# zssjh/stereo-semantic-vo

Measured on AMD Instinct MI355X. Metric: stereo frames/sec on KITTI 00 (full Tracking::Track chain), higher is better.
Workload: dtype u8; 1 GPU; BASELINE configs[2]: synth-kitti00 sequence of 4541 distinct 1241x376 stereo pairs, full Tracking::Track loop per frame (ORB on L and R, sparse stereo, matching passes 1+2, PnP-RANSAC, pose-only LM, map-point lifecycle); ONE sequence per GPU in strict frame order (replicas across GPUs); parallelism=one GPU, resident_pairs_per_gpu=4541, resident_input_bytes_per_gpu=4370984960, frames_tracked=4541, tracker_capacity_flag=0, pnp_samples_through_sequential_fallback=0

## Files before the change

stereo-semantic-vo_amd/csrc/svo_epnp_ord_dev.h:

```cpp
#pragma once
#ifndef HIP_INCLUDE_HIP_HIP_RUNTIME_H
#include <hip/hip_runtime.h>
#endif
#include <stdint.h>

#include "svo_epnp_exact_dev.h"

namespace epnp_ord {

#define EO_FN __device__ __forceinline__
typedef double d2 __attribute__((ext_vector_type(2)));

#include "svo_epnp_ord_tab.h"
#include "svo_epnp_ord_asm.h"

#define EO_SYNC()                                         \
  do {                                                    \
    __builtin_amdgcn_fence(__ATOMIC_ACQ_REL, "wavefront"); \
    __builtin_amdgcn_wave_barrier();                      \
  } while (0)

struct Lds {
  alignas(16) double jr[16 * 16];
  alignas(16) double xch[16][4][4];
  unsigned tab[EO_TAB_TOTAL];
  double pws[16], us[10], alphas[20], cws[12], ccinv[9];
  double M[120];
  double ut4[4][12];
  double L[60], rho[6];
  double sw[3][6];
  double bx[3][6];
  double ccs[3][12], pcs[3][16], abt[3][9], Rc[3][9], rep[3][8];
  alignas(16) double gn[3][6][6];
  double out[3][16];
  int srow[3][6];
  int urow[4];
  double xw[16];
  int flag;
  int sweeps;
  int why;
  long long stamp[8];
#ifdef EO_PROFILE
  long long prof[8];
#endif
};

EO_FN double xdiv(double a, double b) { return a / b; }
EO_FN double xsqrt(double x) { return sqrt(x); }

EO_FN double ndiv(double a, double b) {
  double r = __builtin_amdgcn_rcp(b);
  double e = __builtin_fma(-b, r, 1.0);
  r = __builtin_fma(r, e, r);
  e = __builtin_fma(-b, r, 1.0);
  r = __builtin_fma(r, e, r);
  const double q = a * r;
  const double rem = __builtin_fma(-b, q, a);
  return __builtin_fma(rem, r, q);
}
EO_FN double nsqrt(double x) {
  const double y = __builtin_amdgcn_rsq(x);
  double g = x * y, h = 0.5 * y;
  const double r = __builtin_fma(-h, g, 0.5);
  g = __builtin_fma(g, r, g);
  h = __builtin_fma(h, r, h);
  double d = __builtin_fma(-g, g, x);
  g = __builtin_fma(d, h, g);
  d = __builtin_fma(-g, g, x);
  g = __builtin_fma(d, h, g);
  return g;
}
EO_FN bool w_in_range(double w) { return w >= 7.888609052210118e-31 && w <= 1.2676506002282294e30; }

EO_FN double gsum(double term, double acc) { return __builtin_amdgcn_mfma_f64_4x4x4f64(1.0, term, acc, 0, 0, 0); }
template <int M>
EO_FN double colsum(double t0, double t1, double t2, int g) {
  double acc = gsum(M >= 4 || g < M ? t0 : 0.0, 0.0);
  if (M > 4) acc = gsum(M >= 8 || 4 + g < M ? t1 : 0.0, acc);
  if (M > 8) acc = gsum(M >= 12 || 8 + g < M ? t2 : 0.0, acc);
  return acc;
}

#define EO_TAB3_OFF 0
#define EO_TAB4_OFF (EO_TAB3_OFF + EO_TAB3_STEPS * 3)
#define EO_TAB5_OFF (EO_TAB4_OFF + EO_TAB4_STEPS * 4)
#define EO_TAB12_OFF (EO_TAB5_OFF + EO_TAB5_STEPS * 5)
EO_FN unsigned tab_entry(unsigned e) { return (e & ~16u) | ((e & 16u) << 27); }
EO_FN void load_tables(Lds& S, int lane) {
  for (int e = lane; e < EO_TAB3_STEPS * 3; e += 64) S.tab[EO_TAB3_OFF + e] = tab_entry(c_tab3[0][e]);
  for (int e = lane; e < EO_TAB4_STEPS * 4; e += 64) S.tab[EO_TAB4_OFF + e] = tab_entry(c_tab4[0][e]);
  for (int e = lane; e < EO_TAB5_STEPS * 5; e += 64) S.tab[EO_TAB5_OFF + e] = tab_entry(c_tab5[0][e]);
  for (int e = lane; e < EO_TAB12_STEPS * 12; e += 64) S.tab[EO_TAB12_OFF + e] = tab_entry(c_tab12[0][e]);
}

template <int M>
EO_FN void pair_test(double x0, double x1, double x2, double q0, double q1, double q2, double W, double wP, double mk,
                     double& p, double& thr) {
  const double one = 1.0, eps = 2.220446049250313e-16 * 10;
  double t0, t1, t2, ab, y, g, h, r, d;
  if (M == 12) {
    asm volatile(
        "v_mul_f64 %[t0], %[x0], %[q0]\n\t"
        "v_mul_f64 %[ab], %[W], %[wP]\n\t"
        "v_mul_f64 %[t1], %[x1], %[q1]\n\t"
        "v_mul_f64 %[t2], %[x2], %[q2]\n\t"
        "v_rsq_f64 %[y], %[ab]\n\t"
        "v_mfma_f64_4x4x4_4b_f64 %[p], %[one], %[t0], 0\n\t"
        "v_mul_f64 %[g], %[ab], %[y]\n\t"
        "v_mul_f64 %[h], %[y], 0.5\n\t"
        "v_fma_f64 %[r], -%[h], %[g], 0.5\n\t"
        "v_fma_f64 %[g], %[g], %[r], %[g]\n\t"
        "v_mfma_f64_4x4x4_4b_f64 %[p], %[one], %[t1], %[p]\n\t"
        "v_fma_f64 %[h], %[h], %[r], %[h]\n\t"
        "v_fma_f64 %[d], -%[g], %[g], %[ab]\n\t"
        "v_fma_f64 %[g], %[d], %[h], %[g]\n\t"
        "v_fma_f64 %[d], -%[g], %[g], %[ab]\n\t"
        "v_mfma_f64_4x4x4_4b_f64 %[p], %[one], %[t2], %[p]\n\t"
        "v_fma_f64 %[g], %[d], %[h], %[g]\n\t"
        "v_mul_f64 %[thr], %[g], %[eps]\n\t"
        "s_nop 4"
        : [p] "=&v"(p), [thr] "=&v"(thr), [t0] "=&v"(t0), [t1] "=&v"(t1), [t2] "=&v"(t2), [ab] "=&v"(ab), [y] "=&v"(y),
          [g] "=&v"(g), [h] "=&v"(h), [r] "=&v"(r), [d] "=&v"(d)
        : [x0] "v"(x0), [x1] "v"(x1), [x2] "v"(x2), [q0] "v"(q0), [q1] "v"(q1), [q2] "v"(q2), [W] "v"(W), [wP] "v"(wP),
          [one] "v"(one), [eps] "v"(eps));
  } else if (M == 6) {
    asm volatile(
        "v_mul_f64 %[t0], %[x0], %[q0]\n\t"
        "v_mul_f64 %[t1], %[x1], %[q1]\n\t"
        "v_mul_f64 %[ab], %[W], %[wP]\n\t"
        "v_mul_f64 %[t1], %[t1], %[mk]\n\t"
        "v_rsq_f64 %[y], %[ab]\n\t"
        "v_mfma_f64_4x4x4_4b_f64 %[p], %[one], %[t0], 0\n\t"
        "v_mul_f64 %[g], %[ab], %[y]\n\t"
        "v_mul_f64 %[h], %[y], 0.5\n\t"
        "v_fma_f64 %[r], -%[h], %[g], 0.5\n\t"
        "v_fma_f64 %[g], %[g], %[r], %[g]\n\t"
        "v_mfma_f64_4x4x4_4b_f64 %[p], %[one], %[t1], %[p]\n\t"
        "v_fma_f64 %[h], %[h], %[r], %[h]\n\t"
        "v_fma_f64 %[d], -%[g], %[g], %[ab]\n\t"
        "v_fma_f64 %[g], %[d], %[h], %[g]\n\t"
        "v_fma_f64 %[d], -%[g], %[g], %[ab]\n\t"
        "v_fma_f64 %[g], %[d], %[h], %[g]\n\t"
        "v_mul_f64 %[thr], %[g], %[eps]\n\t"
        "s_nop 0"
        : [p] "=&v"(p), [thr] "=&v"(thr), [t0] "=&v"(t0), [t1] "=&v"(t1), [ab] "=&v"(ab), [y] "=&v"(y), [g] "=&v"(g),
          [h] "=&v"(h), [r] "=&v"(r), [d] "=&v"(d)
        : [x0] "v"(x0), [x1] "v"(x1), [q0] "v"(q0), [q1] "v"(q1), [W] "v"(W), [wP] "v"(wP), [mk] "v"(mk), [one] "v"(one),
          [eps] "v"(eps));
  } else {
    asm volatile(
        "v_mul_f64 %[t0], %[x0], %[q0]\n\t"
        "v_mul_f64 %[ab], %[W], %[wP]\n\t"
        "v_mul_f64 %[t0], %[t0], %[mk]\n\t"
        "v_rsq_f64 %[y], %[ab]\n\t"
        "s_nop 0\n\t"
        "v_mfma_f64_4x4x4_4b_f64 %[p], %[one], %[t0], 0\n\t"
        "v_mul_f64 %[g], %[ab], %[y]\n\t"
        "v_mul_f64 %[h], %[y], 0.5\n\t"
        "v_fma_f64 %[r], -%[h], %[g], 0.5\n\t"
        "v_fma_f64 %[g], %[g], %[r], %[g]\n\t"
        "v_fma_f64 %[h], %[h], %[r], %[h]\n\t"
        "v_fma_f64 %[d], -%[g], %[g], %[ab]\n\t"
        "v_fma_f64 %[g], %[d], %[h], %[g]\n\t"
        "v_fma_f64 %[d], -%[g], %[g], %[ab]\n\t"
        "v_fma_f64 %[g], %[d], %[h], %[g]\n\t"
        "v_mul_f64 %[thr], %[g], %[eps]"
        : [p] "=&v"(p), [thr] "=&v"(thr), [t0] "=&v"(t0), [ab] "=&v"(ab), [y] "=&v"(y), [g] "=&v"(g), [h] "=&v"(h), [r] "=&v"(r),
          [d] "=&v"(d)
        : [x0] "v"(x0), [q0] "v"(q0), [W] "v"(W), [wP] "v"(wP), [mk] "v"(mk), [one] "v"(one), [eps] "v"(eps));
  }
}

template <int M>
EO_FN double row_norm2(double n0, double n1, double n2, double mk) {
  const double one = 1.0;
  double s0, s1, s2, a;
  if (M == 12) {
    asm volatile(
        "v_mul_f64 %[s0], %[n0], %[n0]\n\t"
        "v_mul_f64 %[s1], %[n1], %[n1]\n\t"
        "v_mul_f64 %[s2], %[n2], %[n2]\n\t"
        "v_mfma_f64_4x4x4_4b_f64 %[a], %[one], %[s0], 0\n\t"
        "s_nop 3\n\t"
        "v_mfma_f64_4x4x4_4b_f64 %[a], %[one], %[s1], %[a]\n\t"
        "s_nop 3\n\t"
        "v_mfma_f64_4x4x4_4b_f64 %[a], %[one], %[s2], %[a]\n\t"
        "s_nop 5"
        : [a] "=&v"(a), [s0] "=&v"(s0), [s1] "=&v"(s1), [s2] "=&v"(s2)
        : [n0] "v"(n0), [n1] "v"(n1), [n2] "v"(n2), [one] "v"(one));
  } else if (M == 6) {
    asm volatile(
        "v_mul_f64 %[s0], %[n0], %[n0]\n\t"
        "v_mul_f64 %[s1], %[n1], %[n1]\n\t"
        "v_mul_f64 %[s1], %[s1], %[mk]\n\t"
        "v_mfma_f64_4x4x4_4b_f64 %[a], %[one], %[s0], 0\n\t"
        "s_nop 3\n\t"
        "v_mfma_f64_4x4x4_4b_f64 %[a], %[one], %[s1], %[a]\n\t"
        "s_nop 5"
        : [a] "=&v"(a), [s0] "=&v"(s0), [s1] "=&v"(s1)
        : [n0] "v"(n0), [n1] "v"(n1), [mk] "v"(mk), [one] "v"(one));
  } else {
    asm volatile(
        "v_mul_f64 %[s0], %[n0], %[n0]\n\t"
        "v_mul_f64 %[s0], %[s0], %[mk]\n\t"
        "s_nop 1\n\t"
        "v_mfma_f64_4x4x4_4b_f64 %[a], %[one], %[s0], 0\n\t"
        "s_nop 5"
        : [a] "=&v"(a), [s0] "=&v"(s0)
        : [n0] "v"(n0), [mk] "v"(mk), [one] "v"(one));
  }
  return a;
}

template <int M>
EO_FN unsigned long long jacobi_rows(Lds& S, int n, int base, int lane) {
  const int r = lane & 15, g = lane >> 4, q = r - base;
  const double mk = M == 6 ? (g < 2 ? 1.0 : 0.0) : (M == 3 ? (g < 3 ? 1.0 : 0.0) : 1.0);
  const double eps = 2.220446049250313e-16 * 10;
  double x0 = S.jr[r * 16 + g], x1 = S.jr[r * 16 + 4 + g], x2 = S.jr[r * 16 + 8 + g];
  double* const mine = S.xch[r][g];
  { d2 lo; lo.x = x0; lo.y = x1; *reinterpret_cast<d2*>(mine) = lo; mine[2] = x2; }
  const int tb = n == 12 ? EO_TAB12_OFF : (n == 5 ? EO_TAB5_OFF : (n == 4 ? EO_TAB4_OFF : EO_TAB3_OFF));
  const int steps = n == 12 ? EO_TAB12_STEPS : (n == 5 ? EO_TAB5_STEPS : (n == 4 ? EO_TAB4_STEPS : EO_TAB3_STEPS));
  const int pro = n == 12 ? EO_TAB12_PROLOGUE : (n == 5 ? EO_TAB5_PROLOGUE : (n == 4 ? EO_TAB4_PROLOGUE : EO_TAB3_PROLOGUE));
  static_assert(EO_TAB3_SWEEPS == 1 && EO_TAB4_SWEEPS == 1 && EO_TAB5_SWEEPS == 1 && EO_TAB12_SWEEPS == 1, "one sweep per period");
  auto lds = [](const void* p) { return (unsigned)(unsigned long long)p; };
  const unsigned a_tab = lds(&S.tab[0]);
  const unsigned twrap = a_tab + 4u * (unsigned)(n > 0 ? tb + pro * n + q : 0);
  const unsigned cfg = (unsigned)steps | (unsigned)pro << 8 | (unsigned)(4 * n) << 16;
  const unsigned pm = n > 0 ? ((1u << n) - 1u) << base : 0u;
  EO_SYNC();
  const double eps2 = eps * eps;
  const double eps2hi = eps2 * (1.0 + 9.094947017729282e-13), eps2lo = eps2 * (1.0 - 9.094947017729282e-13);
  unsigned chg = 0, nst = 0, flag = 0;
  int tt = 0, tp = n > 0 ? tb + q : 0, sb = 0;
  const unsigned e0 = S.tab[tp];
  ++tt; tp += n;
  if (tt == steps) { tt = pro; tp = n > 0 ? tb + pro * n + q : 0; ++sb; }
  const unsigned e1 = S.tab[tp];
  const unsigned tpa = a_tab + 4u * (unsigned)tp;
  const unsigned act = n >= 2 ? 1u : 0u;
  const unsigned amine = lds(mine), axch = lds(&S.xch[0][g][0]);
#define EO_JACOBI_OPERANDS                                                                                                       \
  : [x0] "+v"(x0), [x1] "+v"(x1), [x2] "+v"(x2), [chg] "+v"(chg), [nst] "+v"(nst), [flag] "+v"(flag)                              \
  : [e0] "v"(e0), [e1] "v"(e1), [tt] "v"(tt), [tp] "v"(tpa), [sb] "v"(sb), [cfg] "v"(cfg), [twrap] "v"(twrap), [lane] "v"(lane), \
    [base] "v"(base), [act] "v"(act), [pm] "v"(pm), [mk] "v"(mk), [eps] "v"(eps), [eps2hi] "v"(eps2hi), [eps2lo] "v"(eps2lo),   \
    [amine] "v"(amine), [axch] "v"(axch)                                                                                          \
  : EO_JACOBI_ASM_CLOBBERS
  if (M == 12) asm volatile(EO_JACOBI_ASM_12 EO_JACOBI_OPERANDS);
  else if (M == 6) asm volatile(EO_JACOBI_ASM_6 EO_JACOBI_OPERANDS);
  else asm volatile(EO_JACOBI_ASM_3 EO_JACOBI_OPERANDS);
#undef EO_JACOBI_OPERANDS
  const unsigned long long exhausted = __ballot(flag != 0 && n > 0);
  if (M == 12 && flag) S.why |= 1;
  if (M == 12 && lane == 0) S.sweeps = (int)nst;
  const double w = xsqrt(row_norm2<M>(x0, x1, x2, mk));
  const double sc1 = 1 / w;
  if (n > 0) {
    S.jr[r * 16 + g] = M >= 4 || g < M ? x0 * sc1 : x0;
    S.jr[r * 16 + 4 + g] = M >= 8 || 4 + g < M ? x1 * sc1 : x1;
    S.jr[r * 16 + 8 + g] = M >= 12 || 8 + g < M ? x2 * sc1 : x2;
    if (g == 0) S.jr[r * 16 + 15] = w;
  }
  EO_SYNC();
  return exhausted;
}

EO_FN unsigned long long svd_rank(Lds& S, int n, int base, int p, int lane) {
  const int col = lane & 15;
  bool bad = false;
  if (col < n) {
    const double my = S.jr[(base + col) * 16 + 15];
    int rank = 0;
    bad = !w_in_range(my);
    for (int q = 0; q < 5; ++q)
      if (q < n && q != col) {
        const double o = S.jr[(base + q) * 16 + 15];
        rank += o > my ? 1 : 0;
        bad = bad || o == my;
      }
    S.sw[p][rank] = my;
    S.srow[p][rank] = base + col;
  }
  EO_SYNC();
  return __ballot(bad);
}
EO_FN unsigned need_seq(unsigned long long ex, unsigned long long bad) {
  unsigned m = 0;
  for (int p = 0; p < 3; ++p) {
    const unsigned long long rows = 0x001F001F001F001FULL << (5 * p);
    if ((ex & rows) || (bad & (0xFFFFULL << (16 * p)))) m |= 1u << p;
  }
  return m;
}

EO_FN int svd12_smallest(Lds& S, int lane) {
  bool local = false, full = false;
  if (lane < 12) {
    const double my = S.jr[lane * 16 + 15];
    int rank = 0;
    local = my == 0.0;
    full = !w_in_range(my);
    for (int q = 0; q < 12; ++q)
      if (q != lane) {
        const double o = S.jr[q * 16 + 15];
        rank += o > my ? 1 : 0;
        local = local || o == my;
      }
    if (full) S.why |= 2;
    if (rank >= 8) S.urow[11 - rank] = lane;
  }
  const bool any_local = __ballot(local) != 0, any_full = __ballot(full) != 0;
  EO_SYNC();
  if (any_full) return 2;
  if (any_local) return 1;
  if (lane < 48) {
    const int q = lane / 12, k = lane % 12, r = S.urow[q] & 15;
    S.ut4[q][k] = S.jr[r * 16 + k];
  }
  EO_SYNC();
  return 0;
}

__device__ __attribute__((noinline)) void jacobi12_safe(Lds& S, int lane) {
  const double eps = 2.220446049250313e-16 * 10;
  const int r = lane & 15, g = lane >> 4, n = r < 12 ? 12 : 0, q = r;
  double x0 = S.jr[r * 16 + g], x1 = S.jr[r * 16 + 4 + g], x2 = S.jr[r * 16 + 8 + g];
  double W = colsum<12>(x0 * x0, x1 * x1, x2 * x2, g);
  double* const mine = S.xch[r][g];
  mine[0] = x0; mine[1] = x1; mine[2] = x2;
  S.xw[r] = W;
  const int tb = EO_TAB12_OFF, steps = EO_TAB12_STEPS, pro = EO_TAB12_PROLOGUE;
  const unsigned pm = n > 0 ? (1u << 12) - 1u : 0u;
  EO_SYNC();
  int tt = 0, tp = n > 0 ? tb + q : 0, sbase = 0;
  unsigned chg = 0;
  bool active = n >= 2;
  unsigned e = S.tab[tp];
  int nsteps = 0;
  while (__any(active)) {
    int tn = tt + 1, tpn = tp + n, sbn = sbase;
    if (tn == steps) { tn = pro; tpn = tb + pro * n + q; sbn = sbase + 1; }
    const unsigned en = S.tab[n > 0 ? tpn : 0];
    const int pq = e & 15, sw = sbase + (int)((e >> 5) & 3);
    const bool is_j = (e >> 31) != 0;
    const bool valid = active && pq != q && sw < 30;
    const int pr = valid ? pq : r;
    const double* const theirs = S.xch[pr][g];
    const double y0 = theirs[0], y1 = theirs[1], y2 = theirs[2];
    const double p0 = colsum<12>(x0 * y0, x1 * y1, x2 * y2, g);
    const double wP = S.xw[pr];
    const bool rot = valid && !(fabs(p0) <= eps * xsqrt(W * wP));
    if (__any(rot)) {
      const double p = p0 * 2;
      double beta = W - wP;
      if (is_j) beta = -beta;
      double gamma;
      {
        double a = fabs(p), b = fabs(beta);
        if (a > b) { b = xdiv(b, a); gamma = a * xsqrt(1 + b * b); }
        else if (b > 0) { a = xdiv(a, b); gamma = b * xsqrt(1 + a * a); }
        else gamma = 0;
      }
      double c, sn;
      if (beta < 0) {
        const double delta = (gamma - beta) * 0.5;
        sn = xsqrt(xdiv(delta, gamma));
        c = xdiv(p, gamma * sn * 2);
      } else {
        c = xsqrt(xdiv(gamma + beta, gamma * 2));
        sn = xdiv(p, gamma * c * 2);
      }
      const double se = is_j ? -sn : sn;
      const double n0 = c * x0 + se * y0, n1 = c * x1 + se * y1, n2 = c * x2 + se * y2;
      const double Wn = colsum<12>(n0 * n0, n1 * n1, n2 * n2, g);
      EO_SYNC();
      if (rot) {
        x0 = n0; x1 = n1; x2 = n2; W = Wn;
        chg |= 1u << sw;
        mine[0] = x0; mine[1] = x1; mine[2] = x2;
        S.xw[r] = W;
      }
    }
    EO_SYNC();
    const bool closes = active && (e & 0x80u) != 0;
    if (__any(closes)) {
      const int sc = sbase + (int)((e >> 8) & 3);
      const unsigned long long bal = __ballot(closes && ((chg >> (sc & 31)) & 1u));
      if (closes && (sc >= 29 || ((unsigned)bal & pm) == 0u)) active = false;
    }
    tt = tn; tp = tpn; sbase = sbn; e = en;
    ++nsteps;
  }
  if (lane == 0) S.sweeps = 1000000 + nsteps;
  EO_SYNC();
}

typedef __attribute__((address_space(3))) double lds_double;
__device__ __attribute__((noinline)) void svd_small_seq(Lds& S, double* jW, int M, int n, int base, int p) {
  double w[6];
  epnp_exact::jacobi_svd((lds_double*)jW, (lds_double*)&S.jr[base * 16], 16, w, (lds_double*)&S.jr[base * 16 + M], 16, M, n, n);
  for (int i = 0; i < n; ++i) {
    S.sw[p][i] = w[i];
    S.srow[p][i] = base + i;
    S.jr[(base + i) * 16 + 15] = w[i];
  }
  S.flag |= 2; S.why |= 8;
}

__device__ __attribute__((noinline)) void svd12_finish_seq(Lds& S, epnp_exact::Work& xw) {
  for (int i = 0; i < 12; ++i)
    for (int k = 0; k < 12; ++k) xw.ut[i * 12 + k] = S.xch[i][k & 3][k >> 2];
  epnp_exact::jacobi_svd_finish((lds_double*)xw.jW, (lds_double*)xw.ut, 12, xw.d, (lds_double*)nullptr, 0, 12, 12, 12);
  for (int q = 0; q < 4; ++q)
    for (int k = 0; k < 12; ++k) S.ut4[q][k] = xw.ut[(11 - q) * 12 + k];
  S.flag |= 2; S.why |= 4;
}

EO_FN void gauss_newton(Lds& S, int cand, int col, bool owner, const double* L, const double* rho, double* betas) {
  for (int it = 0; it < 5; ++it) {
    double A[6][4], b[6];
    {
      const int i = col < 6 ? col : 0;
      const double* rl = L + 10 * i;
      double* g = S.gn[cand][i];
      const double a0 = 2 * rl[0] * betas[0] + rl[1] * betas[1] + rl[3] * betas[2] + rl[6] * betas[3];
      const double a1 = rl[1] * betas[0] + 2 * rl[2] * betas[1] + rl[4] * betas[2] + rl[7] * betas[3];
      const double a2 = rl[3] * betas[0] + rl[4] * betas[1] + 2 * rl[5] * betas[2] + rl[8] * betas[3];
      const double a3 = rl[6] * betas[0] + rl[7] * betas[1] + rl[8] * betas[2] + 2 * rl[9] * betas[3];
      const double bi = rho[i] - (rl[0] * betas[0] * betas[0] + rl[1] * betas[0] * betas[1] + rl[2] * betas[1] * betas[1] +
                                  rl[3] * betas[0] * betas[2] + rl[4] * betas[1] * betas[2] + rl[5] * betas[2] * betas[2] +
                                  rl[6] * betas[0] * betas[3] + rl[7] * betas[1] * betas[3] + rl[8] * betas[2] * betas[3] +
                                  rl[9] * betas[3] * betas[3]);
      if (owner && col < 6) { g[0] = a0; g[1] = a1; g[2] = a2; g[3] = a3; g[4] = bi; }
    }
    EO_SYNC();
#pragma unroll
    for (int i = 0; i < 6; ++i) {
      const double* g = S.gn[cand][i];
      A[i][0] = g[0]; A[i][1] = g[1]; A[i][2] = g[2]; A[i][3] = g[3]; b[i] = g[4];
    }
    EO_SYNC();
    double A1[4], A2[4], x[4] = {0, 0, 0, 0};
    bool alive = true;
#pragma unroll
    for (int k = 0; k < 4; ++k) {
      double eta = fabs(A[k][k]);
#pragma unroll
      for (int i = k + 1; i < 6; ++i) {
        const double elt = fabs(A[i - 1][k]);
        if (eta < elt) eta = elt;
      }
      if (eta == 0) alive = false;
      const double inv_eta = 1. / eta;
      double sum2 = 0.0;
#pragma unroll
      for (int i = k; i < 6; ++i) {
        A[i][k] *= inv_eta;
        sum2 += A[i][k] * A[i][k];
      }
      double sigma = xsqrt(sum2);
      if (A[k][k] < 0) sigma = -sigma;
      A[k][k] += sigma;
      A1[k] = sigma * A[k][k];
      A2[k] = -eta * sigma;
#pragma unroll
      for (int j = k + 1; j < 4; ++j) {
        double sum = 0;
#pragma unroll
        for (int i = k; i < 6; ++i) sum += A[i][k] * A[i][j];
        const double tau = sum / A1[k];
#pragma unroll
        for (int i = k; i < 6; ++i) A[i][j] -= tau * A[i][k];
      }
    }
#pragma unroll
    for (int j = 0; j < 4; ++j) {
      double tau = 0;
#pragma unroll
      for (int i = j; i < 6; ++i) tau += A[i][j] * b[i];
      tau /= A1[j];
#pragma unroll
      for (int i = j; i < 6; ++i) b[i] -= tau * A[i][j];
    }
    x[3] = b[3] / A2[3];
#pragma unroll
    for (int i = 2; i >= 0; --i) {
      double sum = 0;
#pragma unroll
      for (int j = i + 1; j < 4; ++j) sum += A[i][j] * x[j];
      x[i] = (b[i] - sum) / A2[i];
    }
#pragma unroll
    for (int i = 0; i < 4; ++i) betas[i] += alive ? x[i] : 0.0;
  }
}

EO_FN double dot3(const double* a, const double* b) { return a[0] * b[0] + a[1] * b[1] + a[2] * b[2]; }

EO_FN bool solve5_wave(Lds& S, epnp_exact::Work& xw, const double* K, double* R_out, double* t_out, double* rep, bool force_seq = false) {
  const int lane = threadIdx.x & 63, slot = lane >> 4, col = lane & 15, r16 = lane & 15;
  const double fu = K[0], fv = K[1], uc = K[2], vc = K[3];
  if (lane == 0) { S.flag = force_seq ? 1 : 0; S.why = force_seq ? 16 : 0; S.stamp[0] = clock64(); }
  load_tables(S, lane);
  EO_SYNC();
  if (lane < 3) {
    double c = 0;
    for (int i = 0; i < 5; i++) c += S.pws[3 * i + lane];
    S.cws[lane] = c / 5;
  }
  EO_SYNC();
  auto load_pw0 = [&]() {
    if (lane < 9) {
      const int a = lane / 3, b = lane % 3;
      const double ca = S.cws[a], cb = S.cws[b];
      double s = 0;
      for (int i = 0; i < 5; ++i) s += (S.pws[3 * i + a] - ca) * (S.pws[3 * i + b] - cb);
      S.jr[b * 16 + a] = s;
    } else if (lane < 18) {
      const int r = (lane - 9) / 3, k = (lane - 9) % 3;
      S.jr[r * 16 + 3 + k] = r == k ? 1.0 : 0.0;
    } else if (lane < 36) {
      S.jr[((lane - 18) / 6) * 16 + 6 + (lane - 18) % 6] = 0.0;
    }
    EO_SYNC();
  };
  load_pw0();
  unsigned long long ex = jacobi_rows<3>(S, r16 < 3 ? 3 : 0, r16 < 3 ? 0 : r16, lane);
  unsigned long long bd = svd_rank(S, slot == 0 ? 3 : 0, 0, 0, lane);
  if (ex | bd) {
    load_pw0();
    if (lane == 0) svd_small_seq(S, xw.jW, 3, 3, 0, 0);
    EO_SYNC();
  }
  if (lane < 9) {
    const int i = 1 + lane / 3, j = lane % 3;
    const double k = xsqrt(S.sw[0][i - 1] / 5);
    S.cws[3 * i + j] = S.cws[j] + k * S.jr[S.srow[0][i - 1] * 16 + j];
  }
  EO_SYNC();
  auto load_cc = [&]() {
    if (lane < 9) {
      const int r = lane / 3, k = lane % 3;
      S.jr[r * 16 + k] = S.cws[3 * (r + 1) + k] - S.cws[k];
    } else if (lane < 18) {
      const int r = (lane - 9) / 3, k = (lane - 9) % 3;
      S.jr[r * 16 + 3 + k] = r == k ? 1.0 : 0.0;
    } else if (lane < 36) {
      S.jr[((lane - 18) / 6) * 16 + 6 + (lane - 18) % 6] = 0.0;
    }
    EO_SYNC();
  };
  load_cc();
  ex = jacobi_rows<3>(S, r16 < 3 ? 3 : 0, r16 < 3 ? 0 : r16, lane);
  bd = svd_rank(S, slot == 0 ? 3 : 0, 0, 0, lane);
  if (ex | bd) {
    load_cc();
    if (lane == 0) svd_small_seq(S, xw.jW, 3, 3, 0, 0);
    EO_SYNC();
  }
  if (lane < 9) {
    const int j = lane / 3, c = lane % 3;
    double threshold = 0;
    for (int i = 0; i < 3; ++i) threshold += S.sw[0][i];
    threshold *= 2.220446049250313e-16 * 2;
    double x = 0;
    for (int i = 0; i < 3; ++i) {
      double wi = S.sw[0][i];
      if (fabs(wi) <= threshold) continue;
      wi = 1 / wi;
      const int r = S.srow[0][i];
      double s = S.jr[r * 16 + c];
      s *= wi;
      x = x + s * S.jr[r * 16 + 3 + j];
    }
    S.ccinv[lane] = x;
  }
  EO_SYNC();
  if (lane < 15) {
    const int i = lane / 3, j = lane % 3;
    const double* ci = S.ccinv;
    const double* pi = S.pws + 3 * i;
    S.alphas[4 * i + 1 + j] = ci[3 * j] * (pi[0] - S.cws[0]) + ci[3 * j + 1] * (pi[1] - S.cws[1]) + ci[3 * j + 2] * (pi[2] - S.cws[2]);
  }
  EO_SYNC();
  if (lane < 5) {
    const double* a = S.alphas + 4 * lane;
    S.alphas[4 * lane] = 1.0f - a[1] - a[2] - a[3];
  }
  EO_SYNC();
  if (lane == 0) S.stamp[1] = clock64();
  for (int e = lane; e < 120; e += 64) {
    const int r = e / 12, cc = e % 12, i = r >> 1, q = cc / 3, t = cc % 3;
    const double as = S.alphas[4 * i + q], u = S.us[2 * i], v = S.us[2 * i + 1];
    double m;
    if (r & 1) m = t == 0 ? 0.0 : (t == 1 ? as * fv : as * (vc - v));
    else m = t == 0 ? as * fu : (t == 1 ? 0.0 : as * (uc - u));
    S.M[e] = m;
  }
  EO_SYNC();
  auto load_mtm = [&]() {
    for (int e = lane; e < 144; e += 64) {
      const int a = e / 12, b = e % 12;
      double s = 0;
      for (int r = 0; r < 10; ++r) s += S.M[12 * r + a] * S.M[12 * r + b];
      S.jr[b * 16 + a] = s;
    }
    EO_SYNC();
  };
  load_mtm();
  if (lane == 0) S.stamp[2] = clock64();
  const bool degenerate = (S.why & 8) != 0;
  unsigned long long ex12 = 0;
  int fin12 = 2;
  if (!degenerate) {
    ex12 = jacobi_rows<12>(S, r16 < 12 ? 12 : 0, r16 < 12 ? 0 : r16, lane);
    fin12 = svd12_smallest(S, lane);
  }
  if (ex12 || fin12) {
    if (ex12 || fin12 == 2) {
      if (!degenerate) load_mtm();
      jacobi12_safe(S, lane);
    }
    if (lane == 0) svd12_finish_seq(S, xw);
    EO_SYNC();
  }
  if (lane == 0) S.stamp[3] = clock64();
  if (lane < 60) {
    const int i = lane / 10, c = lane % 10;
    const int pa = i < 3 ? 0 : (i < 5 ? 1 : 2), pb = i < 3 ? i + 1 : (i < 5 ? i - 1 : 3);
    const int y = c >= 6 ? 3 : (c >= 3 ? 2 : (c >= 1 ? 1 : 0)), x = c - y * (y + 1) / 2;
    double dx[3], dy[3];
    for (int k = 0; k < 3; ++k) {
      dx[k] = S.ut4[x][3 * pa + k] - S.ut4[x][3 * pb + k];
      dy[k] = S.ut4[y][3 * pa + k] - S.ut4[y][3 * pb + k];
    }
    const double d = dot3(dx, dy);
    S.L[lane] = x == y ? d : 2.0f * d;
  }
  if (lane < 6) {
    const int pa = lane < 3 ? 0 : (lane < 5 ? 1 : 2), pb = lane < 3 ? lane + 1 : (lane < 5 ? lane - 1 : 3);
    const double* p1 = S.cws + 3 * pa;
    const double* p2 = S.cws + 3 * pb;
    S.rho[lane] = (p1[0] - p2[0]) * (p1[0] - p2[0]) + (p1[1] - p2[1]) * (p1[1] - p2[1]) + (p1[2] - p2[2]) * (p1[2] - p2[2]);
  }
  EO_SYNC();
  const int cand = slot < 3 ? slot : 0;
  const int nc = slot == 0 ? 4 : (slot == 1 ? 3 : (slot == 2 ? 5 : 0));
  const int base = 5 * cand;
  auto load_l = [&](int only) {
    if (slot < 3 && (only < 0 || slot == only)) {
      for (int i = 0; i < nc; ++i) {
        const int lc = slot == 0 ? (i == 2 ? 3 : (i == 3 ? 6 : i)) : i;
        double v = 0.0;
        if (col < 6) v = S.L[10 * col + lc];
        else if (col - 6 == i) v = 1.0;
        S.jr[(base + i) * 16 + col] = v;
      }
    }
    EO_SYNC();
  };
  load_l(-1);
  {
    const int pc = r16 / 5, pn = pc == 0 ? 4 : (pc == 1 ? 3 : 5);
    const bool mine = r16 < 15 && r16 % 5 < pn;
    ex = jacobi_rows<6>(S, mine ? pn : 0, mine ? 5 * pc : r16, lane);
  }
  bd = svd_rank(S, nc, base, cand, lane);
  if (ex | bd) {
    const unsigned need = need_seq(ex, bd);
    for (int pp = 0; pp < 3; ++pp)
      if (need >> pp & 1) load_l(pp);
    if (slot < 3 && col == 0 && (need >> slot & 1)) svd_small_seq(S, slot == 0 ? xw.jW : (slot == 1 ? xw.sA : xw.sUt), 6, nc, base, cand);
    EO_SYNC();
  }
  if (slot < 3 && col < nc) {
    double threshold = 0;
    for (int i = 0; i < nc; ++i) threshold += S.sw[cand][i];
    threshold *= 2.220446049250313e-16 * 2;
    double x = 0;
    for (int i = 0; i < nc; ++i) {
      double wi = S.sw[cand][i];
      if (fabs(wi) <= threshold) continue;
      wi = 1 / wi;
      const int r = S.srow[cand][i];
      double s = 0;
      for (int k = 0; k < 6; ++k) s += S.jr[r * 16 + k] * S.rho[k];
      s *= wi;
      x = x + s * S.jr[r * 16 + 6 + col];
    }
    S.bx[cand][col] = x;
  }
  EO_SYNC();
  if (lane == 0) S.stamp[4] = clock64();
  double betas[4];
  {
    const double* bx = S.bx[cand];
    const double b0 = bx[0], b1 = bx[1], b2 = bx[2], b3 = bx[3];
    if (slot == 0) {
      if (b0 < 0) { betas[0] = xsqrt(-b0); betas[1] = -b1 / betas[0]; betas[2] = -b2 / betas[0]; betas[3] = -b3 / betas[0]; }
      else { betas[0] = xsqrt(b0); betas[1] = b1 / betas[0]; betas[2] = b2 / betas[0]; betas[3] = b3 / betas[0]; }
    } else {
      if (b0 < 0) { betas[0] = xsqrt(-b0); betas[1] = (b2 < 0) ? xsqrt(-b2) : 0.0; }
      else { betas[0] = xsqrt(b0); betas[1] = (b2 > 0) ? xsqrt(b2) : 0.0; }
      if (b1 < 0) betas[0] = -betas[0];
      betas[2] = slot == 2 ? b3 / betas[0] : 0.0;
      betas[3] = 0.0;
    }
  }
  {
    double rho[6];
    for (int k = 0; k < 6; ++k) rho[k] = S.rho[k];
    gauss_newton(S, cand, col, slot < 3, S.L, rho, betas);
  }
  if (lane == 0) S.stamp[5] = clock64();
  if (slot < 3 && col < 12) {
    double c = 0.0;
    for (int i = 0; i < 4; ++i) c += betas[i] * S.ut4[i][col];
    S.ccs[cand][col] = c;
  }
  EO_SYNC();
  if (slot < 3 && col < 15) {
    const int i = col / 3, j = col % 3;
    const double* a = S.alphas + 4 * i;
    const double* cc = S.ccs[cand];
    S.pcs[cand][col] = a[0] * cc[j] + a[1] * cc[3 + j] + a[2] * cc[6 + j] + a[3] * cc[9 + j];
  }
  EO_SYNC();
  double pc0[3], pw0[3];
  bool flip;
  {
    const double* pc = S.pcs[cand];
    flip = pc[2] < 0.0;
    for (int j = 0; j < 3; ++j) { pc0[j] = 0; pw0[j] = 0; }
    for (int i = 0; i < 5; ++i)
      for (int j = 0; j < 3; ++j) { pc0[j] += flip ? -pc[3 * i + j] : pc[3 * i + j]; pw0[j] += S.pws[3 * i + j]; }
    for (int j = 0; j < 3; ++j) { pc0[j] /= 5; pw0[j] /= 5; }
  }
  auto load_abt = [&](int only) {
    const double* pc = S.pcs[cand];
    if (slot < 3 && (only < 0 || slot == only) && col < 9) {
      const int j = col / 3, k = col % 3;
      double s = 0;
      for (int i = 0; i < 5; ++i) s += ((flip ? -pc[3 * i + j] : pc[3 * i + j]) - pc0[j]) * (S.pws[3 * i + k] - pw0[k]);
      S.jr[(base + k) * 16 + j] = s;
    } else if (slot < 3 && (only < 0 || slot == only) && col < 12) {
      const int r = col - 9;
      for (int k = 0; k < 3; ++k) S.jr[(base + r) * 16 + 3 + k] = r == k ? 1.0 : 0.0;
      for (int k = 6; k < 12; ++k) S.jr[(base + r) * 16 + k] = 0.0;
    }
    EO_SYNC();
  };
  load_abt(-1);
  {
    const bool mine = r16 < 15 && r16 % 5 < 3;
    ex = jacobi_rows<3>(S, mine ? 3 : 0, mine ? 5 * (r16 / 5) : r16, lane);
  }
  bd = svd_rank(S, slot < 3 ? 3 : 0, base, cand, lane);
  if (ex | bd) {
    const unsigned need = need_seq(ex, bd);
    for (int pp = 0; pp < 3; ++pp)
      if (need >> pp & 1) load_abt(pp);
    if (slot < 3 && col == 0 && (need >> slot & 1)) svd_small_seq(S, slot == 0 ? xw.jW : (slot == 1 ? xw.sA : xw.sUt), 3, 3, base, cand);
    EO_SYNC();
  }
  if (slot < 3 && col < 9) {
    const int i = col / 3, j = col % 3;
    const int r0 = S.srow[cand][0], r1 = S.srow[cand][1], r2 = S.srow[cand][2];
    S.Rc[cand][col] = S.jr[r0 * 16 + i] * S.jr[r0 * 16 + 3 + j] + S.jr[r1 * 16 + i] * S.jr[r1 * 16 + 3 + j] + S.jr[r2 * 16 + i] * S.jr[r2 * 16 + 3 + j];
  }
  EO_SYNC();
  double R[9], t[3];
  for (int k = 0; k < 9; ++k) R[k] = S.Rc[cand][k];
  {
    const double det = R[0] * R[4] * R[8] + R[1] * R[5] * R[6] + R[2] * R[3] * R[7] - R[2] * R[4] * R[6] - R[1] * R[3] * R[8] - R[0] * R[5] * R[7];
    if (det < 0) { R[6] = -R[6]; R[7] = -R[7]; R[8] = -R[8]; }
  }
  t[0] = pc0[0] - dot3(R, pw0); t[1] = pc0[1] - dot3(R + 3, pw0); t[2] = pc0[2] - dot3(R + 6, pw0);
  if (slot < 3 && col < 5) {
    const double* pw = S.pws + 3 * col;
    const double Xc = dot3(R, pw) + t[0], Yc = dot3(R + 3, pw) + t[1], inv_Zc = 1.0 / (dot3(R + 6, pw) + t[2]);
    const double ue = uc + fu * Xc * inv_Zc, ve = vc + fv * Yc * inv_Zc;
    const double u = S.us[2 * col], v = S.us[2 * col + 1];
    S.rep[cand][col] = xsqrt((u - ue) * (u - ue) + (v - ve) * (v - ve));
  }
  EO_SYNC();
  if (slot < 3 && col == 0) {
    double sum2 = 0.0;
    for (int i = 0; i < 5; ++i) sum2 += S.rep[cand][i];
    double* o = S.out[cand];
    for (int k = 0; k < 9; ++k) o[k] = R[k];
    o[9] = t[0]; o[10] = t[1]; o[11] = t[2];
    o[12] = sum2 / 5;
  }
  EO_SYNC();
  if (lane == 0) S.stamp[6] = clock64();
  bool fin = true;
  if (S.flag & 1) {
    if (lane == 0) {
      double* x5 = xw.PW0;
      double* u5 = xw.gA;
      for (int i = 0; i < 15; ++i) x5[i] = S.pws[i];
      for (int i = 0; i < 10; ++i) u5[i] = S.us[i];
      double Rx[9], tx[3], rx[3];
      const bool ok = epnp_exact::solve5(xw, x5, u5, K, Rx, tx, rx);
      for (int k = 0; k < 9; ++k) S.out[0][k] = Rx[k];
      for (int k = 0; k < 3; ++k) S.out[0][9 + k] = tx[k];
      S.out[0][12] = rx[0]; S.out[1][12] = rx[1]; S.out[2][12] = rx[2];
      S.out[0][13] = ok ? 1.0 : 0.0;
    }
    EO_SYNC();
    for (int k = 0; k < 9; ++k) R_out[k] = S.out[0][k];
    for (int k = 0; k < 3; ++k) t_out[k] = S.out[0][9 + k];
    fin = S.out[0][13] != 0.0;
  } else {
    int N = 0;
    if (S.out[1][12] < S.out[0][12]) N = 1;
    if (S.out[2][12] < S.out[N][12]) N = 2;
    for (int k = 0; k < 9; ++k) { R_out[k] = S.out[N][k]; fin = fin && isfinite(S.out[N][k]); }
    for (int k = 0; k < 3; ++k) { t_out[k] = S.out[N][9 + k]; fin = fin && isfinite(S.out[N][9 + k]); }
  }
  if (rep) { rep[0] = S.out[0][12]; rep[1] = S.out[1][12]; rep[2] = S.out[2][12]; }
  if (lane == 0) S.stamp[7] = clock64();
  EO_SYNC();
  return fin;
}

}
```

Measured before the change: 9537 stereo frames/s.

## Distribute Gauss-Newton QR across row lanes with DPP broadcasts instead of LDS

Replaces the per-lane redundant Gauss-Newton 6x4 QR solve, which exchanged its rows through LDS with wave barriers each iteration, with a lane-distributed formulation. Each of the first lanes in a 16-lane row owns one column of A (or b), and pivot data is broadcast with DPP row_newbcast. This removes the LDS scratch array and the two syncs per iteration and spreads the QR arithmetic across lanes. It adds a host-side bitwise checker so the lane version can be compared against a reference. The risk is precision or ordering differences from the original serial code, plus extra broadcast instructions.

```diff
diff --git a/stereo-semantic-vo_amd/csrc/svo_epnp_ord_dev.h b/stereo-semantic-vo_amd/csrc/svo_epnp_ord_dev.h
--- a/stereo-semantic-vo_amd/csrc/svo_epnp_ord_dev.h
+++ b/stereo-semantic-vo_amd/csrc/svo_epnp_ord_dev.h
@@ -5,6 +5,7 @@
 #include <stdint.h>
 
 #include "svo_epnp_exact_dev.h"
+#include "svo_lanes.h"
 
 namespace epnp_ord {
 
@@ -31,7 +32,6 @@
   double sw[3][6];
   double bx[3][6];
   double ccs[3][12], pcs[3][16], abt[3][9], Rc[3][9], rep[3][8];
-  alignas(16) double gn[3][6][6];
   double out[3][16];
   int srow[3][6];
   int urow[4];
@@ -417,83 +417,28 @@
   S.flag |= 2; S.why |= 4;
 }
 
-EO_FN void gauss_newton(Lds& S, int cand, int col, bool owner, const double* L, const double* rho, double* betas) {
-  for (int it = 0; it < 5; ++it) {
-    double A[6][4], b[6];
-    {
-      const int i = col < 6 ? col : 0;
-      const double* rl = L + 10 * i;
-      double* g = S.gn[cand][i];
-      const double a0 = 2 * rl[0] * betas[0] + rl[1] * betas[1] + rl[3] * betas[2] + rl[6] * betas[3];
-      const double a1 = rl[1] * betas[0] + 2 * rl[2] * betas[1] + rl[4] * betas[2] + rl[7] * betas[3];
-      const double a2 = rl[3] * betas[0] + rl[4] * betas[1] + 2 * rl[5] * betas[2] + rl[8] * betas[3];
-      const double a3 = rl[6] * betas[0] + rl[7] * betas[1] + rl[8] * betas[2] + 2 * rl[9] * betas[3];
-      const double bi = rho[i] - (rl[0] * betas[0] * betas[0] + rl[1] * betas[0] * betas[1] + rl[2] * betas[1] * betas[1] +
-                                  rl[3] * betas[0] * betas[2] + rl[4] * betas[1] * betas[2] + rl[5] * betas[2] * betas[2] +
-                                  rl[6] * betas[0] * betas[3] + rl[7] * betas[1] * betas[3] + rl[8] * betas[2] * betas[3] +
-                                  rl[9] * betas[3] * betas[3]);
-      if (owner && col < 6) { g[0] = a0; g[1] = a1; g[2] = a2; g[3] = a3; g[4] = bi; }
-    }
-    EO_SYNC();
+struct RowDpp {
+  typedef double real;
+  typedef bool mask;
+  int col;
+  EO_FN double c(double d) const { return d; }
+  EO_FN double abs(double a) const { return fabs(a); }
+  EO_FN double sqrt(double a) const { return xsqrt(a); }
+  EO_FN bool lt(double a, double b) const { return a < b; }
+  EO_FN bool eq(double a, double b) const { return a == b; }
+  EO_FN double sel(bool m, double a, double b) const { return m ? a : b; }
+  EO_FN bool land(bool a, bool b) const { return a && b; }
+  EO_FN bool lnot(bool a) const { return !a; }
+  EO_FN bool lane_is(int l) const { return col == l; }
+  template <int K>
+  EO_FN double bcast(double v) const { return __builtin_amdgcn_update_dpp(v, v, 0x150 + K, 0xf, 0xf, false); }
+};
+EO_FN void gauss_newton(const Lds& S, int col, double* betas) {
+  const RowDpp x{col};
+  double coef[svo_lanes::GN_NCOEF];
 #pragma unroll
-    for (int i = 0; i < 6; ++i) {
-      const double* g = S.gn[cand][i];
-      A[i][0] = g[0]; A[i][1] = g[1]; A[i][2] = g[2]; A[i][3] = g[3]; b[i] = g[4];
-    }
-    EO_SYNC();
-    double A1[4], A2[4], x[4] = {0, 0, 0, 0};
-    bool alive = true;
-#pragma unroll
-    for (int k = 0; k < 4; ++k) {
-      double eta = fabs(A[k][k]);
-#pragma unroll
-      for (int i = k + 1; i < 6; ++i) {
-        const double elt = fabs(A[i - 1][k]);
-        if (eta < elt) eta = elt;
-      }
-      if (eta == 0) alive = false;
-      const double inv_eta = 1. / eta;
-      double sum2 = 0.0;
-#pragma unroll
-      for (int i = k; i < 6; ++i) {
-        A[i][k] *= inv_eta;
-        sum2 += A[i][k] * A[i][k];
-      }
-      double sigma = xsqrt(sum2);
-      if (A[k][k] < 0) sigma = -sigma;
-      A[k][k] += sigma;
-      A1[k] = sigma * A[k][k];
-      A2[k] = -eta * sigma;
-#pragma unroll
-      for (int j = k + 1; j < 4; ++j) {
-        double sum = 0;
-#pragma unroll
-        for (int i = k; i < 6; ++i) sum += A[i][k] * A[i][j];
-        const double tau = sum / A1[k];
-#pragma unroll
-        for (int i = k; i < 6; ++i) A[i][j] -= tau * A[i][k];
-      }
-    }
-#pragma unroll
-    for (int j = 0; j < 4; ++j) {
-      double tau = 0;
-#pragma unroll
-      for (int i = j; i < 6; ++i) tau += A[i][j] * b[i];
-      tau /= A1[j];
-#pragma unroll
-      for (int i = j; i < 6; ++i) b[i] -= tau * A[i][j];
-    }
-    x[3] = b[3] / A2[3];
-#pragma unroll
-    for (int i = 2; i >= 0; --i) {
-      double sum = 0;
-#pragma unroll
-      for (int j = i + 1; j < 4; ++j) sum += A[i][j] * x[j];
-      x[i] = (b[i] - sum) / A2[i];
-    }
-#pragma unroll
-    for (int i = 0; i < 4; ++i) betas[i] += alive ? x[i] : 0.0;
-  }
+  for (int e = 0; e < svo_lanes::GN_NCOEF; ++e) coef[e] = svo_lanes::gn_lane_coef(S.L, S.rho, col, e);
+  svo_lanes::gauss_newton_lanes(x, coef, betas);
 }
 
 EO_FN double dot3(const double* a, const double* b) { return a[0] * b[0] + a[1] * b[1] + a[2] * b[2]; }
@@ -708,11 +653,7 @@
       betas[3] = 0.0;
     }
   }
-  {
-    double rho[6];
-    for (int k = 0; k < 6; ++k) rho[k] = S.rho[k];
-    gauss_newton(S, cand, col, slot < 3, S.L, rho, betas);
-  }
+  gauss_newton(S, col, betas);
   if (lane == 0) S.stamp[5] = clock64();
   if (slot < 3 && col < 12) {
     double c = 0.0;
diff --git a/stereo-semantic-vo_amd/csrc/svo_lanes.h b/stereo-semantic-vo_amd/csrc/svo_lanes.h
--- /dev/null
+++ b/stereo-semantic-vo_amd/csrc/svo_lanes.h
@@ -0,0 +1,127 @@
+#pragma once
+
+#if defined(__HIPCC__)
+#define SVO_LANES_FN __device__ __forceinline__
+#define SVO_LANES_UNROLL _Pragma("unroll")
+#else
+#define SVO_LANES_FN inline __attribute__((always_inline))
+#define SVO_LANES_UNROLL
+#endif
+
+namespace svo_lanes {
+
+constexpr int GN_NCOEF = 24;
+SVO_LANES_FN int gn_lane_coef_index(int col, int e) {
+  const int i = e >> 2, j = e & 3, a = col < j ? col : j, b = col < j ? j : col;
+  const int in_a = 10 * i + b * (b + 1) / 2 + a;
+  const int row = col - 4;
+  const int in_b = e < 10 ? 10 * row + e : (e == 10 ? 60 + row : -1);
+  return col < 4 ? in_a : (col < 10 ? in_b : -1);
+}
+SVO_LANES_FN bool gn_lane_coef_doubled(int col, int e) { return col < 4 && (e & 3) == col; }
+SVO_LANES_FN double gn_lane_coef(const double* L, const double* rho, int col, int e) {
+  const int idx = gn_lane_coef_index(col, e);
+  const double* src = idx >= 60 ? rho + (idx - 60) : L + (idx < 0 ? 0 : idx);
+  double v = *src;
+  if (idx < 0) v = 0.0;
+  return gn_lane_coef_doubled(col, e) ? 2 * v : v;
+}
+
+template <class X>
+SVO_LANES_FN void gn_build_lanes(const X& x, const typename X::real* coef, const typename X::real* betas, typename X::real* v) {
+  typedef typename X::real R;
+  const R b0 = betas[0], b1 = betas[1], b2 = betas[2], b3 = betas[3];
+  R acol[6];
+SVO_LANES_UNROLL
+  for (int i = 0; i < 6; ++i) acol[i] = coef[4 * i] * b0 + coef[4 * i + 1] * b1 + coef[4 * i + 2] * b2 + coef[4 * i + 3] * b3;
+  const R bi = coef[10] - (coef[0] * b0 * b0 + coef[1] * b0 * b1 + coef[2] * b1 * b1 + coef[3] * b0 * b2 + coef[4] * b1 * b2 +
+                           coef[5] * b2 * b2 + coef[6] * b0 * b3 + coef[7] * b1 * b3 + coef[8] * b2 * b3 + coef[9] * b3 * b3);
+  const typename X::mask is_b = x.lane_is(4);
+  v[0] = x.sel(is_b, x.template bcast<4>(bi), acol[0]);
+  v[1] = x.sel(is_b, x.template bcast<5>(bi), acol[1]);
+  v[2] = x.sel(is_b, x.template bcast<6>(bi), acol[2]);
+  v[3] = x.sel(is_b, x.template bcast<7>(bi), acol[3]);
+  v[4] = x.sel(is_b, x.template bcast<8>(bi), acol[4]);
+  v[5] = x.sel(is_b, x.template bcast<9>(bi), acol[5]);
+}
+
+template <int K, class X>
+SVO_LANES_FN void qr_step_lanes(const X& x, typename X::real* v, typename X::real* A2, typename X::mask& alive) {
+  typedef typename X::real R;
+  R eta = x.abs(v[K]);
+SVO_LANES_UNROLL
+  for (int i = K + 1; i < 6; ++i) {
+    const R elt = x.abs(v[i - 1]);
+    eta = x.sel(x.lt(eta, elt), elt, eta);
+  }
+  const R inv_eta = x.c(1.) / eta;
+  R c[6];
+  R sum2 = x.c(0.0);
+SVO_LANES_UNROLL
+  for (int i = K; i < 6; ++i) {
+    c[i] = v[i] * inv_eta;
+    sum2 = sum2 + c[i] * c[i];
+  }
+  R sigma = x.sqrt(sum2);
+  sigma = x.sel(x.lt(c[K], x.c(0.0)), -sigma, sigma);
+  c[K] = c[K] + sigma;
+  const R a1 = sigma * c[K];
+  const R a2 = -eta * sigma;
+  const R etak = x.template bcast<K>(eta);
+  const R a1k = x.template bcast<K>(a1);
+  A2[K] = x.template bcast<K>(a2);
+  R ck[6];
+SVO_LANES_UNROLL
+  for (int i = K; i < 6; ++i) ck[i] = x.template bcast<K>(c[i]);
+  alive = x.land(alive, x.lnot(x.eq(etak, x.c(0.0))));
+  R sum = x.c(0.0);
+SVO_LANES_UNROLL
+  for (int i = K; i < 6; ++i) sum = sum + ck[i] * v[i];
+  const R tau = sum / a1k;
+SVO_LANES_UNROLL
+  for (int i = K; i < 6; ++i) v[i] = v[i] - tau * ck[i];
+}
+
+template <class X>
+SVO_LANES_FN void qr_solve_lanes(const X& x, typename X::real* v, typename X::real* xs) {
+  typedef typename X::real R;
+  R A2[4];
+  typename X::mask alive = x.eq(x.c(0.0), x.c(0.0));
+  qr_step_lanes<0>(x, v, A2, alive);
+  qr_step_lanes<1>(x, v, A2, alive);
+  qr_step_lanes<2>(x, v, A2, alive);
+  qr_step_lanes<3>(x, v, A2, alive);
+  const R q0 = x.template bcast<4>(v[0]), q1 = x.template bcast<4>(v[1]), q2 = x.template bcast<4>(v[2]), q3 = x.template bcast<4>(v[3]);
+  const R a01 = x.template bcast<1>(v[0]);
+  const R a02 = x.template bcast<2>(v[0]), a12 = x.template bcast<2>(v[1]);
+  const R a03 = x.template bcast<3>(v[0]), a13 = x.template bcast<3>(v[1]), a23 = x.template bcast<3>(v[2]);
+  const R x3 = q3 / A2[3];
+  R sum = x.c(0.0);
+  sum = sum + a23 * x3;
+  const R x2 = (q2 - sum) / A2[2];
+  sum = x.c(0.0);
+  sum = sum + a12 * x2;
+  sum = sum + a13 * x3;
+  const R x1 = (q1 - sum) / A2[1];
+  sum = x.c(0.0);
+  sum = sum + a01 * x1;
+  sum = sum + a02 * x2;
+  sum = sum + a03 * x3;
+  const R x0 = (q0 - sum) / A2[0];
+  const R zero = x.c(0.0);
+  xs[0] = x.sel(alive, x0, zero); xs[1] = x.sel(alive, x1, zero); xs[2] = x.sel(alive, x2, zero); xs[3] = x.sel(alive, x3, zero);
+}
+
+template <class X>
+SVO_LANES_FN void gauss_newton_lanes(const X& x, const typename X::real* coef, typename X::real* betas) {
+  typedef typename X::real R;
+  for (int it = 0; it < 5; ++it) {
+    R v[6], xs[4];
+    gn_build_lanes(x, coef, betas, v);
+    qr_solve_lanes(x, v, xs);
+SVO_LANES_UNROLL
+    for (int i = 0; i < 4; ++i) betas[i] = betas[i] + xs[i];
+  }
+}
+
+}
diff --git a/stereo-semantic-vo_amd/host/lane_check.cc b/stereo-semantic-vo_amd/host/lane_check.cc
--- /dev/null
+++ b/stereo-semantic-vo_amd/host/lane_check.cc
@@ -0,0 +1,86 @@
+#include <cinttypes>
+#include <cmath>
+#include <cstdint>
+#include <cstdio>
+#include <cstring>
+#include <vector>
+
+#include "../csrc/svo_lanes.h"
+
+namespace {
+
+constexpr int NL = 16;
+struct Lanes { double l[NL]; };
+struct Mask { bool l[NL]; };
+#define LANEWISE(expr) do { for (int i = 0; i < NL; ++i) r.l[i] = (expr); } while (0)
+inline Lanes operator+(const Lanes& a, const Lanes& b) { Lanes r; LANEWISE(a.l[i] + b.l[i]); return r; }
+inline Lanes operator-(const Lanes& a, const Lanes& b) { Lanes r; LANEWISE(a.l[i] - b.l[i]); return r; }
+inline Lanes operator*(const Lanes& a, const Lanes& b) { Lanes r; LANEWISE(a.l[i] * b.l[i]); return r; }
+inline Lanes operator/(const Lanes& a, const Lanes& b) { Lanes r; LANEWISE(a.l[i] / b.l[i]); return r; }
+inline Lanes operator-(const Lanes& a) { Lanes r; LANEWISE(-a.l[i]); return r; }
+
+struct RowHost {
+  typedef Lanes real;
+  typedef Mask mask;
+  Lanes c(double d) const { Lanes r; LANEWISE(d); return r; }
+  Lanes abs(const Lanes& a) const { Lanes r; LANEWISE(std::fabs(a.l[i])); return r; }
+  Lanes sqrt(const Lanes& a) const { Lanes r; LANEWISE(std::sqrt(a.l[i])); return r; }
+  Mask lt(const Lanes& a, const Lanes& b) const { Mask r; LANEWISE(a.l[i] < b.l[i]); return r; }
+  Mask eq(const Lanes& a, const Lanes& b) const { Mask r; LANEWISE(a.l[i] == b.l[i]); return r; }
+  Lanes sel(const Mask& m, const Lanes& a, const Lanes& b) const { Lanes r; LANEWISE(m.l[i] ? a.l[i] : b.l[i]); return r; }
+  Mask land(const Mask& a, const Mask& b) const { Mask r; LANEWISE(a.l[i] && b.l[i]); return r; }
+  Mask lnot(const Mask& a) const { Mask r; LANEWISE(!a.l[i]); return r; }
+  Mask lane_is(int l) const { Mask r; LANEWISE(i == l); return r; }
+  template <int K>
+  Lanes bcast(const Lanes& a) const { Lanes r; LANEWISE(a.l[K]); return r; }
+};
+
+uint64_t bits(double d) { uint64_t u; std::memcpy(&u, &d, 8); return u; }
+bool read_case(double* v, int n) {
+  for (int i = 0; i < n; ++i) {
+    uint64_t u;
+    if (std::scanf("%" SCNx64, &u) != 1) return false;
+    std::memcpy(&v[i], &u, 8);
+  }
+  return true;
+}
+void print4(char tag, const double* x) {
+  std::printf("%c %016" PRIx64 " %016" PRIx64 " %016" PRIx64 " %016" PRIx64 "\n", tag, bits(x[0]), bits(x[1]), bits(x[2]), bits(x[3]));
+}
+bool gather4(const Lanes* r, double* out) {
+  bool same = true;
+  for (int k = 0; k < 4; ++k) {
+    out[k] = r[k].l[0];
+    for (int i = 1; i < NL; ++i) same = same && bits(r[k].l[i]) == bits(out[k]);
+  }
+  return same;
+}
+
+}
+
+int main(int argc, char** argv) {
+  const bool qr = argc > 1 && !std::strcmp(argv[1], "qr"), gn = argc > 1 && !std::strcmp(argv[1], "gn");
+  if (!qr && !gn) { std::fprintf(stderr, "usage: lane_check qr|gn < cases\n"); return 2; }
+  const RowHost x;
+  int status = 0, n = 0;
+  double in[70], lanes_out[4];
+  while (read_case(in, qr ? 30 : 70)) {
+    if (qr) {
+      Lanes v[6], xs[4];
+      for (int i = 0; i < 6; ++i)
+        for (int l = 0; l < NL; ++l) v[i].l[l] = l < 4 ? in[4 * i + l] : (l == 4 ? in[24 + i] : 0.0);
+      svo_lanes::qr_solve_lanes(x, v, xs);
+      if (!gather4(xs, lanes_out)) { std::printf("D %d\n", n); status = 1; }
+    } else {
+      Lanes coef[svo_lanes::GN_NCOEF], betas[4];
+      for (int e = 0; e < svo_lanes::GN_NCOEF; ++e)
+        for (int l = 0; l < NL; ++l) coef[e].l[l] = svo_lanes::gn_lane_coef(in, in + 60, l, e);
+      for (int k = 0; k < 4; ++k) betas[k] = x.c(in[66 + k]);
+      svo_lanes::gauss_newton_lanes(x, coef, betas);
+      if (!gather4(betas, lanes_out)) { std::printf("D %d\n", n); status = 1; }
+    }
+    print4('L', lanes_out);
+    ++n;
+  }
+  return status;
+}
```

After: 9667 stereo frames/s, median of 6. 1.4% higher.
